# micropilot/myosuite-mjx

Measured on AMD Instinct MI355X. Metric: env-steps/s (whole node) myoHandPoseRandom-v0 batch 4096, higher is better.
Workload: dtype f32

## Files before the change

### myosuite_mjx_amd/csrc/myo_kernel_wave.h

```cpp
#ifndef MYO_KERNEL_WAVE_H
#define MYO_KERNEL_WAVE_H

#define NCONW 32
#define MPRW 14
static_assert(4 * MPRW <= 63, "the scheduler carries the table in a 64-word row (word 63 = entry count)");
struct LayW {
  int qpos, qvel, act, ctrl, lpos, lmat, axis, anchor, xv, qfc, sq, mprw, X;
  int tJ, tlen, tforce;
  int cdof, cinert, crb, cvel, cacc, cfrc;
  int gpos, gax, cand, cdist, cpos, cnrm, cpair, cJ, cdofs;
  int Mp;
  int tJp;
  int total;
};
__host__ __device__ constexpr LayW layout_w(int nq, int nv, int nu, int nl, int ngt, int maxnnz, int ncg, bool has_tl, int nvt, int kc, int nc, int nj) {
  LayW Y{};
  int o = 0;
  Y.qpos = o; o += nq; Y.qvel = o; o += nv; Y.act = o; o += nu; Y.ctrl = o; o += nu;
  Y.lpos = o; o += 3 * nl; Y.lmat = o; o += 9 * nl; Y.axis = o; o += 3 * nv; Y.anchor = o; o += 3 * nv;
  Y.xv = o; o += nvt; Y.qfc = o; o += nvt; Y.sq = o; o += nvt * (nvt + 1); Y.mprw = o; o += 4 * MPRW;
  Y.tJp = 0;
  if (has_tl) { Y.tJp = o; o += ngt * maxnnz + 2 * ngt; }
  Y.X = o;
  Y.tJ = o; o += ngt * maxnnz; Y.tlen = o; o += ngt; Y.tforce = o; o += nu;
  const int endT = o;
  o = Y.X;
  Y.cdof = o; o += 6 * nv; Y.cinert = o; o += 10 * nl; Y.crb = o; o += 10 * nl; Y.cvel = o; o += 6 * nl; Y.cacc = o; o += 6 * nl; Y.cfrc = o; o += 6 * nl;
  const int endD = o;
  o = Y.X;
  Y.Mp = o;
  Y.gpos = o; o += 3 * ncg; Y.gax = o; o += 3 * ncg;
  Y.cand = o; o += NCAND;
  if (o - Y.Mp < (nvt * (nvt + 1)) / 2) o = Y.Mp + (nvt * (nvt + 1)) / 2;
  Y.cdist = o; o += nc; Y.cpos = o; o += 3 * nc; Y.cnrm = o; o += 3 * nc; Y.cpair = o; o += nc;
  Y.cJ = o; o += nc * nj * kc; Y.cdofs = o; o += nc * ((kc + 3) / 4);
  if (o < endT) o = endT;
  if (o < endD) o = endD;
  Y.total = o;
  return Y;
}
struct HfDev { int on, nrow, ncol, cg; float size[4], pos[3]; };
struct DevModelW {
  LayW lay;
  gpi seg_order, seg_tendon, gt_dl;
  gpf link_mat0;
  int nwrapseg, ndl, has_tl;
  gpf tl;
  int nq, has_free, neq;
  int has_j0;
  gpf gt_j0;
  HfDev hf;
  gpi link_free, dof_qposadr, eq_i, link_chain_adr, link_chain;
  int kin_dnmax;
  gpi kin_base, kin_adr, kin_vec;
  gpf eq_f;
  gpf mesh_rec, mesh_startrec, mesh_aabb;
  gpf fl, mesh_vert;
  gpf4 seg_rec;
  gpi dl_pk;
  gpf4 cg_rec;
  gpf4 pair_rec;
  gpi pair_dl_pk;
  gpi kin_pk;
  int kin_nround;
  gpi link_desc;
  gpi link_adof;
  gpi dof_anc;
  unsigned int free_rot[2], free_j3[2];
};
#define SEGR 9
#ifndef MPR_TOL
#define MPR_TOL 1e-8f
#endif

__device__ __forceinline__ float rdlane(float v, int l) { return __int_as_float(__builtin_amdgcn_readlane(__float_as_int(v), l)); }
__device__ __forceinline__ int rdlanei(int v, int l) { return __builtin_amdgcn_readlane(v, l); }
__device__ __forceinline__ float uniformf(float v) { return __int_as_float(__builtin_amdgcn_readfirstlane(__float_as_int(v))); }
template <int CTRL> __device__ __forceinline__ float dpp_add(float v) {
  return v + __int_as_float(__builtin_amdgcn_update_dpp(0, __float_as_int(v), CTRL, 0xf, 0xf, true));
}
__device__ __forceinline__ float wave_sum(float v) {
  v = dpp_add<0xB1>(v);
  v = dpp_add<0x4E>(v);
  v = dpp_add<0x141>(v);
  v = dpp_add<0x140>(v);
  return (rdlane(v, 0) + rdlane(v, 16)) + (rdlane(v, 32) + rdlane(v, 48));
}
#define WFOR(i, n) for (int i = lane; i < (n); i += 64)
__device__ __forceinline__ int wave_lane() {
  int l;
  asm volatile("v_mbcnt_lo_u32_b32 %0, -1, 0\n\tv_mbcnt_hi_u32_b32 %0, -1, %0" : "=v"(l));
  return l;
}
#define CDOF(E_, Y_, c_, k_) ((int)((((const unsigned int*)((E_) + (Y_).cdofs))[CDW * (c_) + ((k_) >> 2)] >> (8 * ((k_) & 3))) & 255u))
#define CDOFP(W_, k_) ((int)(((W_)[(k_) >> 2] >> (8 * ((k_) & 3))) & 255u))

template <int NVT> __device__ __forceinline__ float chol_rows(float (&r)[NVT], int lane) {
  float invd = 1.0f;
#pragma unroll
  for (int j = 0; j < NVT; j++) {
    const float pj = fmaxf(rdlane(r[j], j), MINVALF);
    const float ip = __builtin_amdgcn_rcpf(pj);
    const float col = lane > j ? r[j] : 0.f;
    const float lt = col * ip;
    r[j] = lt;
    if (lane == j) invd = ip;
#pragma unroll
    for (int k = j + 1; k < NVT; k++) r[k] -= lt * rdlane(col, k);
  }
  return invd;
}
template <int SPEC> struct SpecTree { static constexpr int nv = 0; static constexpr int parent[1] = {-1}; };
template <> struct SpecTree<1> { static constexpr int nv = 23;
  static constexpr int parent[23] = {-1, 0, 1, 2, 3, 4, 5, 2, 7, 8, 9, 2, 11, 12, 13, 2, 15, 16, 17, 2, 19, 20, 21}; };
template <> struct SpecTree<2> { static constexpr int nv = 34;
  static constexpr int parent[34] = {-1, 0, 1, 2, 3, 4, 5, 6, 7, 8, 9, 10, 11, 12, 13, 14, 15, 8, 17, 18, 5, 20, 21, 22, 23, 24, 25, 26, 27, 28, 29, 22, 31, 32}; };
template <> struct SpecTree<3> : SpecTree<2> {};
template <int SPEC> __host__ __device__ constexpr bool tree_anc(int a, int d) {
  int p = SpecTree<SPEC>::parent[d];
  while (p >= 0) { if (p == a) return true; p = SpecTree<SPEC>::parent[p]; }
  return false;
}
template <int NVT, int SPEC, int J, int K> __device__ __forceinline__ void tree_update(float (&r)[NVT], float lt, float col) {
  constexpr int nv = SpecTree<SPEC>::nv;
  if constexpr (K > J && J < nv && K < nv) {
    if constexpr (tree_anc<SPEC>(nv - 1 - K, nv - 1 - J)) r[K] -= lt * rdlane(col, K);
  }
}
template <int NVT, int SPEC, int J, int... Ks> __device__ __forceinline__ void tree_col(float (&r)[NVT], float lt, float col, std::integer_sequence<int, Ks...>) {
  (tree_update<NVT, SPEC, J, Ks>(r, lt, col), ...);
}
template <int NVT, int SPEC, int J> __device__ __forceinline__ void tree_step(float (&r)[NVT], float& invd, int lane) {
  const float pj = fmaxf(rdlane(r[J], J), MINVALF);
  const float ip = __builtin_amdgcn_rcpf(pj);
  const float col = lane > J ? r[J] : 0.f;
  const float lt = col * ip;
  r[J] = lt;
  if (lane == J) invd = ip;
  tree_col<NVT, SPEC, J>(r, lt, col, std::make_integer_sequence<int, NVT>{});
}
template <int NVT, int SPEC, int... Js> __device__ __forceinline__ void tree_all(float (&r)[NVT], float& invd, int lane, std::integer_sequence<int, Js...>) {
  (tree_step<NVT, SPEC, Js>(r, invd, lane), ...);
}
template <int NVT, int SPEC> __device__ __forceinline__ float chol_rows_tree(float (&r)[NVT], int lane) {
  float invd = 1.0f;
  tree_all<NVT, SPEC>(r, invd, lane, std::make_integer_sequence<int, NVT>{});
  return invd;
}
template <int NVT> __device__ __forceinline__ float chol_solve_rows(const float (&r)[NVT], float invd, float b, const float* T, int lane) {
  float y = b;
#pragma unroll
  for (int j = 0; j < NVT; j++) y = fmaf(-r[j], rdlane(y, j), y);
  y *= invd;
  const float* Tc = T + (lane < NVT ? lane : 0);
#pragma unroll
  for (int j = NVT - 1; j >= 0; j--) y = fmaf(-Tc[j * (NVT + 1)], rdlane(y, j), y);
  return y;
}
template <int NVT> __device__ __forceinline__ float symv_lds(const float* Mp, float x, int lane, int nv) {
  float s = 0;
  const int d = lane < nv ? lane : 0;
  const int based = (d * (d + 1)) / 2;
#pragma unroll
  for (int k = 0; k < NVT; k++) {
    int kk = k < nv ? k : 0;
    int adr = (kk <= d) ? based + kk : (kk * (kk + 1)) / 2 + d;
    float mv = (k < nv && lane < nv) ? Mp[adr] : 0.f;
    s += mv * rdlane(x, k);
  }
// ... 1179 lines not shown
          lD = __builtin_amdgcn_rcpf(R);
        }
      }
    }
    float caref[NR], cD = 0.f, cmu = 0.f;
#pragma unroll
    for (int k = 0; k < NR; k++) caref[k] = 0.f;
    float cmut = 0.f, cD2 = 0.f;
    int ckc = 0;
    constexpr int ROWS = 8 + NJ * KC + CDW;
    enum { S_AREF = 0, S_D = NR, S_MU = NR + 1, S_MUT = NR + 2, S_D2 = NR + 3, S_KC = NR + 4, S_JAR = NR + 5, S_JV = 2 * NR + 5, S_FC = 3 * NR + 5, S_HC = 3 * NR + 9, S_SIG = 3 * NR + 16 };
    static_assert(!TRK || 3 * NR + 17 <= TRK_STATE, "state block of a second-bank contact");
    const bool bank1 = TRK && ncon > 64;
    auto st1 = [&](int c) -> float* { return ovf_env + (size_t)(c - NC) * ovf_row + ROWS; };
    const bool b1lane = bank1 && lane + 64 < ncon;
    int nefc_b1 = 0;
    auto build_row = [&](const float* pdist, const float* ppos, const float* pnrm, const int* ppair, float* cJ, unsigned int* cdw) {
      const int cw_ = ppair[0], p = cw_ & 2047;
      const float4 pq0_ = W.pair_rec[4 * (size_t)(p)]; const int pw_ = __float_as_int(pq0_.x); const int P[6] = {pw_ & 255, (pw_ >> 8) & 255, (int)((unsigned int)cw_ >> 16), (cw_ >> 11) & 31, (pw_ >> 16) & 15, (pw_ >> 20) & 15};
      const float* F = M.pair_f + 12 * p;
      float n[3] = {pnrm[0], pnrm[1], pnrm[2]}, t1[3], t2[3];
      float cp[3] = {ppos[0], ppos[1], ppos[2]};
      make_frame(n, t1, t2);
      if (FULL && P[4] == 2) {
        const float* ax = E + Y.gax + 3 * P[1];
        float t = dot3(ax, n), y[3] = {ax[0] - t * n[0], ax[1] - t * n[1], ax[2] - t * n[2]};
        float yn = norm3(y);
        if (yn >= 0.5f) {
          float inv = 1.0f / yn;
          t1[0] = y[0] * inv; t1[1] = y[1] * inv; t1[2] = y[2] * inv;
          cross3(t2, n, t1);
        }
      }
      float vn = 0, vt1 = 0, vt2 = 0, vs = 0;
      unsigned int dpk[CDW];
#pragma unroll
      for (int k = 0; k < CDW; k++) dpk[k] = 0;
      ckc = P[3];
#pragma unroll
      for (int k = 0; k < KC; k++) {
        float jn = 0, j1 = 0, j2 = 0, js = 0;
        int d = 0;
        if (k < ckc) {
          const int de_ = W.pair_dl_pk[P[2] + k];
          d = de_ & 127;
          float sg = (float)(de_ >> 8);
          const float* ax = E + Y.axis + 3 * d;
          float col[3];
          if (de_ & 128) {
            float r[3] = {cp[0] - E[Y.anchor + 3 * d], cp[1] - E[Y.anchor + 3 * d + 1], cp[2] - E[Y.anchor + 3 * d + 2]};
            cross3(col, ax, r);
          } else { col[0] = ax[0]; col[1] = ax[1]; col[2] = ax[2]; }
          jn = sg * dot3(n, col); j1 = sg * dot3(t1, col); j2 = sg * dot3(t2, col);
          float qv = E[Y.qvel + d];
          vn += jn * qv; vt1 += j1 * qv; vt2 += j2 * qv;
          if constexpr (TRK) { js = (de_ & 128) ? sg * dot3(n, ax) : 0.f; vs += js * qv; }
        }
        cJ[k] = jn; cJ[KC + k] = j1; cJ[2 * KC + k] = j2;
        if constexpr (TRK) cJ[3 * KC + k] = js;
        dpk[k >> 2] |= (unsigned int)d << (8 * (k & 3));
      }
#pragma unroll
      for (int k = 0; k < CDW; k++) cdw[k] = dpk[k];
      float dist = pdist[0], incl = F[0] - F[1];
      cmu = F[2];
      float imp = impedance(F + 6, dist, incl), K, B;
      kbi(F[4], F[5], F[7], M.timestep, &K, &B);
      if (FULL && P[5] == 1) {
        cmu = 0.f;
        cD = 0.25f / fmaxf(MINVALF, (1 - imp) / imp * F[3]);
      } else {
        float R0 = fmaxf(MINVALF, (1 - imp) / imp * F[3] * (1 + cmu * cmu));
        cD = __builtin_amdgcn_rcpf(fmaxf(MINVALF, 2 * cmu * cmu * R0));
      }
      float pos = -K * imp * (dist - incl);
      caref[0] = -B * (vn + cmu * vt1) + pos; caref[1] = -B * (vn - cmu * vt1) + pos;
      caref[2] = -B * (vn + cmu * vt2) + pos; caref[3] = -B * (vn - cmu * vt2) + pos;
      if constexpr (TRK) {
        if (P[5] == 4) { cmut = F[11]; cD2 = cD; caref[4] = -B * (vn + cmut * vs) + pos; caref[5] = -B * (vn - cmut * vs) + pos; }
      }
    };
    if constexpr (KC == 8 && !FULL && !TRK) {
      float vn_c = 0.f, vt1_c = 0.f, vt2_c = 0.f;
      const int rg = lane >> 3, rk = lane & 7;
      for (int c0 = 0; c0 < ncon; c0 += 8) {
        const int c = c0 + rg;
        float pv0 = 0.f, pv1 = 0.f, pv2 = 0.f;
        auto row_cols = [&](const float* ppos, const float* pnrm, const int* ppair, float* cJ, unsigned int* cdw) {
          const int cw_ = ppair[0];
          const int P[4] = {0, 0, (int)((unsigned int)cw_ >> 16), (cw_ >> 11) & 31};
          const float n[3] = {pnrm[0], pnrm[1], pnrm[2]}, cp[3] = {ppos[0], ppos[1], ppos[2]};
          float t1[3], t2[3];
          make_frame(n, t1, t2);
          float jn = 0.f, j1 = 0.f, j2 = 0.f;
          int d = 0;
          if (rk < P[3]) {
            const int de_ = W.pair_dl_pk[P[2] + rk];
            d = de_ & 127;
            const float sg = (float)(de_ >> 8);
            const float* ax = E + Y.axis + 3 * d;
            float col[3];
            if (de_ & 128) {
              const float r[3] = {cp[0] - E[Y.anchor + 3 * d], cp[1] - E[Y.anchor + 3 * d + 1], cp[2] - E[Y.anchor + 3 * d + 2]};
              cross3(col, ax, r);
            } else { col[0] = ax[0]; col[1] = ax[1]; col[2] = ax[2]; }
            jn = sg * dot3(n, col); j1 = sg * dot3(t1, col); j2 = sg * dot3(t2, col);
            const float qv = E[Y.qvel + d];
            pv0 = jn * qv; pv1 = j1 * qv; pv2 = j2 * qv;
          }
          cJ[rk] = jn; cJ[KC + rk] = j1; cJ[2 * KC + rk] = j2;
          ((unsigned char*)cdw)[rk] = (unsigned char)d;
        };
        if (c < ncon) {
          if (c < NC) row_cols(E + Y.cpos + 3 * c, E + Y.cnrm + 3 * c, (const int*)(E + Y.cpair) + c, E + Y.cJ + c * NJ * KC, (unsigned int*)(E + Y.cdofs) + CDW * c);
          else { float* g = ovf_env + (c - NC) * ovf_row; row_cols(g + 1, g + 4, (const int*)g + 7, g + 8, (unsigned int*)(g + 8 + NJ * KC)); }
        }
#pragma unroll
        for (int m_ = 1; m_ < 8; m_ <<= 1) { pv0 += __shfl_xor(pv0, m_); pv1 += __shfl_xor(pv1, m_); pv2 += __shfl_xor(pv2, m_); }
        const int src = (8 * (lane - c0)) & 63;
        const float a0 = __shfl(pv0, src), a1 = __shfl(pv1, src), a2 = __shfl(pv2, src);
        if (lane >= c0 && lane < c0 + 8) { vn_c = a0; vt1_c = a1; vt2_c = a2; }
      }
      SYNC();
      if (lane < ncon) {
        const float* g = lane < NC ? nullptr : ovf_env + (lane - NC) * ovf_row;
        const int cw_ = lane < NC ? ((const int*)(E + Y.cpair))[lane] : ((const int*)g)[7], p = cw_ & 2047;
        const float dist = lane < NC ? E[Y.cdist + lane] : g[0];
        const float* F = M.pair_f + 12 * p;
        ckc = (cw_ >> 11) & 31;
        const float incl = F[0] - F[1];
        cmu = F[2];
        float imp = impedance(F + 6, dist, incl), K, B;
        kbi(F[4], F[5], F[7], M.timestep, &K, &B);
        const float R0 = fmaxf(MINVALF, (1 - imp) / imp * F[3] * (1 + cmu * cmu));
        cD = __builtin_amdgcn_rcpf(fmaxf(MINVALF, 2 * cmu * cmu * R0));
        const float pos = -K * imp * (dist - incl);
        caref[0] = -B * (vn_c + cmu * vt1_c) + pos; caref[1] = -B * (vn_c - cmu * vt1_c) + pos;
        caref[2] = -B * (vn_c + cmu * vt2_c) + pos; caref[3] = -B * (vn_c - cmu * vt2_c) + pos;
      }
    } else if constexpr (KC == 20) {
      const int rg = lane / KC, rk = lane - rg * KC;
      float vn_c = 0.f, vt1_c = 0.f, vt2_c = 0.f, vs_c = 0.f;
      float vn_1 = 0.f, vt1_1 = 0.f, vt2_1 = 0.f, vs_1 = 0.f;
      for (int c0 = 0; c0 < ncon; c0 += 3) {
        if (lane < 12) E[Y.xv + lane] = 0.f;
        SYNC();
        const int c = c0 + rg;
        auto row_cols = [&](const float* ppos, const float* pnrm, const int* ppair, float* cJ, unsigned int* cdw) {
          const int cw_ = ppair[0];
          const float4 pq0_ = W.pair_rec[4 * (size_t)(cw_ & 2047)]; const int pw_ = __float_as_int(pq0_.x); const int P[6] = {pw_ & 255, (pw_ >> 8) & 255, (int)((unsigned int)cw_ >> 16), (cw_ >> 11) & 31, (pw_ >> 16) & 15, (pw_ >> 20) & 15};
          const float n[3] = {pnrm[0], pnrm[1], pnrm[2]}, cp[3] = {ppos[0], ppos[1], ppos[2]};
          float t1[3], t2[3];
          make_frame(n, t1, t2);
          if (P[4] == 2) {
            const float* ax = E + Y.gax + 3 * P[1];
            float t = dot3(ax, n), y[3] = {ax[0] - t * n[0], ax[1] - t * n[1], ax[2] - t * n[2]};
            float yn = norm3(y);
            if (yn >= 0.5f) {
              float inv = 1.0f / yn;
              t1[0] = y[0] * inv; t1[1] = y[1] * inv; t1[2] = y[2] * inv;
              cross3(t2, n, t1);
            }
          }
          float jn = 0.f, j1 = 0.f, j2 = 0.f, js = 0.f;
          int d = 0;
          if (rk < P[3]) {
            const int de_ = W.pair_dl_pk[P[2] + rk];
            d = de_ & 127;
            const float sg = (float)(de_ >> 8);
            const float* ax = E + Y.axis + 3 * d;
            float col[3];
            const bool hinge = (de_ & 128) != 0;
            if (hinge) {
              const float r[3] = {cp[0] - E[Y.anchor + 3 * d], cp[1] - E[Y.anchor + 3 * d + 1], cp[2] - E[Y.anchor + 3 * d + 2]};
              cross3(col, ax, r);
            } else { col[0] = ax[0]; col[1] = ax[1]; col[2] = ax[2]; }
            jn = sg * dot3(n, col); j1 = sg * dot3(t1, col); j2 = sg * dot3(t2, col);
            const float qv = E[Y.qvel + d];
            atomicAdd(&E[Y.xv + 4 * rg], jn * qv); atomicAdd(&E[Y.xv + 4 * rg + 1], j1 * qv); atomicAdd(&E[Y.xv + 4 * rg + 2], j2 * qv);
            if constexpr (TRK) { js = hinge ? sg * dot3(n, ax) : 0.f; atomicAdd(&E[Y.xv + 4 * rg + 3], js * qv); }
          }
          cJ[rk] = jn; cJ[KC + rk] = j1; cJ[2 * KC + rk] = j2;
          if constexpr (TRK) cJ[3 * KC + rk] = js;
          ((unsigned char*)cdw)[rk] = (unsigned char)d;
        };
        if (rg < 3 && c < ncon) {
          if (c < NC) row_cols(E + Y.cpos + 3 * c, E + Y.cnrm + 3 * c, (const int*)(E + Y.cpair) + c, E + Y.cJ + c * NJ * KC, (unsigned int*)(E + Y.cdofs) + CDW * c);
          else { float* g = ovf_env + (c - NC) * ovf_row; row_cols(g + 1, g + 4, (const int*)g + 7, g + 8, (unsigned int*)(g + 8 + NJ * KC)); }
        }
        SYNC();
        if (lane >= c0 && lane < c0 + 3) { const int g = lane - c0; vn_c = E[Y.xv + 4 * g]; vt1_c = E[Y.xv + 4 * g + 1]; vt2_c = E[Y.xv + 4 * g + 2]; vs_c = E[Y.xv + 4 * g + 3]; }
        if constexpr (TRK) {
          if (b1lane && lane + 64 >= c0 && lane + 64 < c0 + 3) { const int g = lane + 64 - c0; vn_1 = E[Y.xv + 4 * g]; vt1_1 = E[Y.xv + 4 * g + 1]; vt2_1 = E[Y.xv + 4 * g + 2]; vs_1 = E[Y.xv + 4 * g + 3]; }
        }
        SYNC();
      }
      auto row_consts = [&](const int cc, const float vn_c, const float vt1_c, const float vt2_c, const float vs_c, float (&caref)[NR], float& cD, float& cmu, float& cmut,
                            float& cD2, int& ckc) {
        const int lane = cc;
        const float* g = lane < NC ? nullptr : ovf_env + (lane - NC) * ovf_row;
        const int cw_ = lane < NC ? ((const int*)(E + Y.cpair))[lane] : ((const int*)g)[7], p = cw_ & 2047;
        const float dist = lane < NC ? E[Y.cdist + lane] : g[0];
        const float4 pq0_ = W.pair_rec[4 * (size_t)(p)]; const int pw_ = __float_as_int(pq0_.x); const int P[6] = {pw_ & 255, (pw_ >> 8) & 255, __float_as_int(pq0_.w), (pw_ >> 24) & 255, (pw_ >> 16) & 15, (pw_ >> 20) & 15};
// ... 76 lines not shown
        }
      }
      unsigned long long bal = __ballot(tact);
      int slot = nt + __popcll(bal & ((1ull << lane) - 1ull));
      const int ntcap = min(nct, 64);
      if (tact && slot < ntcap) {
        float* const row = slot < NC ? nullptr : ovf_env + (slot - NC) * ovf_row;
        float* cJ = slot < NC ? E + Y.cJ + slot * NJ * KC : row + 8;
        unsigned int dpk[CDW];
#pragma unroll
        for (int k = 0; k < CDW; k++) dpk[k] = 0;
        int kc = 0;
#pragma unroll
        for (int k = 0; k < KC; k++) {
          int d = k < maxnnz_ ? M.gt_dofs[gt * maxnnz_ + k] : -1;
          float jv = d >= 0 ? t_sign * E[Y.tJp + gt * maxnnz_ + k] : 0.f;
          if (d >= 0) kc = k + 1; else d = 0;
          cJ[k] = jv; cJ[KC + k] = 0.f; cJ[2 * KC + k] = 0.f;
          if constexpr (TRK) cJ[3 * KC + k] = 0.f;
          dpk[k >> 2] |= (unsigned int)d << (8 * (k & 3));
        }
        unsigned int* const dw = slot < NC ? (unsigned int*)(E + Y.cdofs) + CDW * slot : (unsigned int*)(row + 8 + NJ * KC);
#pragma unroll
        for (int k = 0; k < CDW; k++) dw[k] = dpk[k];
        if (slot < NC) { E[Y.cdist + slot] = t_aref; E[Y.cpos + 3 * slot] = t_D; E[Y.cpos + 3 * slot + 1] = (float)kc; }
        else { row[0] = t_aref; row[1] = t_D; row[2] = (float)kc; }
      }
      nt += __popcll(bal);
      }
      if (nt > min(nct, 64)) { flags |= MYO_FLAG_CONTACT_OVERFLOW; nt = min(nct, 64); }
      SYNC();
      if (lane >= ncon && lane < nt) {
        const float* const row = lane < NC ? nullptr : ovf_env + (lane - NC) * ovf_row;
        const float a = lane < NC ? E[Y.cdist + lane] : row[0];
        caref[0] = caref[1] = caref[2] = caref[3] = a;
        cD = 0.25f * (lane < NC ? E[Y.cpos + 3 * lane] : row[1]); cmu = 0.f; ckc = (int)(lane < NC ? E[Y.cpos + 3 * lane + 1] : row[2]);
      }
      nefc += nt - ncon;
      ncon = nt;
    }
    float eJ2 = 0.f, eD = 0.f, earef = 0.f, ejar = 0.f, ejv = 0.f;
    int ed1 = 0, ed2 = 0;
    const bool eact = lane < neq;
    if (eact) {
      const int* Q = W.eq_i + 4 * lane;
      const float* F = W.eq_f + 16 * lane;
      ed1 = Q[0]; ed2 = Q[1];
      float x = E[Y.qpos + Q[3]] - F[6];
      float pos = E[Y.qpos + Q[2]] - F[5] - (F[0] + x * (F[1] + x * (F[2] + x * (F[3] + x * F[4]))));
      eJ2 = -(F[1] + x * (2 * F[2] + x * (3 * F[3] + x * 4 * F[4])));
      float vel = E[Y.qvel + ed1] + eJ2 * E[Y.qvel + ed2];
      float imp = impedance(F + 9, pos, 0.f), K, B;
      kbi(F[7], F[8], F[10], M.timestep, &K, &B);
      earef = -B * vel - K * imp * pos;
      eD = __builtin_amdgcn_rcpf(fmaxf(MINVALF, (1 - imp) / imp * F[14]));
    }
    nefc += neq;
    SYNC();
#ifdef MYO_NO_MROW
    constexpr bool MROW = false;
#else
    constexpr bool MROW = NVT > 24 && !RK4;
#endif
    float mrow[MROW ? NVT : 1];
    if constexpr (MROW) {
      const int ml = lane < nv ? lane : 0;
#pragma unroll
      for (int k = 0; k < NVT; k++) mrow[k] = lane < nv ? E[Y.sq + ml * (NVT + 1) + k] : 0.f;
    }
    if (lane < nv) {
      const int based = (lane * (lane + 1)) / 2;
#pragma unroll
      for (int k = 0; k < NVT; k++) if (k <= lane) E[Y.Mp + based + k] = E[Y.sq + lane * (NVT + 1) + k];
    }
    const float* Mp = E + Y.Mp;
    auto symv_reg = [&](float x, int lane) -> float {
      if constexpr (MROW) {
        float s0 = 0.f, s1 = 0.f;
#pragma unroll
        for (int k = 0; k < NVT; k += 2) { s0 = fmaf(mrow[k], rdlane(x, k), s0); if (k + 1 < NVT) s1 = fmaf(mrow[k + 1], rdlane(x, k + 1), s1); }
        return s0 + s1;
      } else return symv_lds<NVT>(Mp, x, lane, nv);
    };
    SYNC();
    STAMP(5);
    SUB0();
    float Ma = 0.f, grad = 0.f, qfc = 0.f, ljar = 0.f, ljv = 0.f, cost = 0.f, qaccE = 0.f, qacc = 0.f;
    float cjar[NR], cjv[NR];
#pragma unroll
    for (int k = 0; k < NR; k++) { cjar[k] = 0.f; cjv[k] = 0.f; }
    int phase = nefc > 0 ? 0 : 1, iters = 0;
    if (phase == 0) {
      qacc = warm_r;
      Ma = symv_reg(qacc, lane);
      ljar = lsign * qacc - laref;
      if constexpr (TRK) fljar = qacc - flaref;
      if (lane < nv) E[Y.xv + lane] = qacc;
      SYNC();
      auto row_jar = [&](const float* cJ, const unsigned int* cdw) {
        float an = 0, a1 = 0, a2 = 0, a3 = 0;
#pragma unroll
        for (int k = 0; k < KC; k++) {
          float xv = E[Y.xv + CDOFP(cdw, k)]; an += cJ[k] * xv; a1 += cJ[KC + k] * xv; a2 += cJ[2 * KC + k] * xv;
          if constexpr (TRK) a3 += cJ[3 * KC + k] * xv;
        }
        cjar[0] = an + cmu * a1 - caref[0]; cjar[1] = an - cmu * a1 - caref[1]; cjar[2] = an + cmu * a2 - caref[2]; cjar[3] = an - cmu * a2 - caref[3];
        if constexpr (TRK) { cjar[4] = an + cmut * a3 - caref[4]; cjar[5] = an - cmut * a3 - caref[5]; }
      };
      if (lane < ncon) {
        if (lane < NC) row_jar(E + Y.cJ + lane * NJ * KC, (const unsigned int*)(E + Y.cdofs) + CDW * lane);
        else { const float* g = ovf_env + (lane - NC) * ovf_row; row_jar(g + 8, (const unsigned int*)(g + 8 + NJ * KC)); }
      }
      if constexpr (TRK) {
        if (b1lane) {
          const float* g = ovf_env + (lane + 64 - NC) * ovf_row;
          const unsigned int* cdw = (const unsigned int*)(g + 8 + NJ * KC);
          float* S = st1(lane + 64);
          float an = 0, a1 = 0, a2 = 0, a3 = 0;
          for (int k = 0; k < KC; k++) { const float xv = E[Y.xv + CDOFP(cdw, k)]; an += g[8 + k] * xv; a1 += g[8 + KC + k] * xv; a2 += g[8 + 2 * KC + k] * xv; a3 += g[8 + 3 * KC + k] * xv; }
          const float mu = S[S_MU], mut = S[S_MUT];
          S[S_JAR] = an + mu * a1 - S[S_AREF]; S[S_JAR + 1] = an - mu * a1 - S[S_AREF + 1]; S[S_JAR + 2] = an + mu * a2 - S[S_AREF + 2]; S[S_JAR + 3] = an - mu * a2 - S[S_AREF + 3];
          S[S_JAR + 4] = an + mut * a3 - S[S_AREF + 4]; S[S_JAR + 5] = an - mut * a3 - S[S_AREF + 5];
        }
      }
      if (eact) ejar = E[Y.xv + ed1] + eJ2 * E[Y.xv + ed2] - earef;
    }
    SUB(6);
    bool first = true;
    int sig_prev = -1;
    while (true) {
      const int lane = wave_lane();
      float r[NVT], rhs, invd;
      bool refactor = true;
      if (phase == 0) {
        bool lact = lsign != 0.f && ljar < 0;
        float w0 = cjar[0] < 0 ? cD : 0.f, w1 = cjar[1] < 0 ? cD : 0.f, w2 = cjar[2] < 0 ? cD : 0.f, w3 = cjar[3] < 0 ? cD : 0.f;
        float f0 = -w0 * cjar[0], f1 = -w1 * cjar[1], f2 = -w2 * cjar[2], f3 = -w3 * cjar[3];
        float w4 = 0.f, w5 = 0.f, f4 = 0.f, f5 = 0.f, flforce = 0.f, flcost = 0.f;
        bool flquad = false;
        if constexpr (TRK) {
          w4 = cjar[4] < 0 ? cD2 : 0.f; w5 = cjar[5] < 0 ? cD2 : 0.f;
          f4 = -w4 * cjar[4]; f5 = -w5 * cjar[5];
          if (flf > 0.f) {
            if (fljar <= -flrf) { flforce = flf; flcost = flf * (-0.5f * flrf - fljar); }
            else if (fljar >= flrf) { flforce = -flf; flcost = flf * (-0.5f * flrf + fljar); }
            else { flforce = -flD * fljar; flcost = 0.5f * flD * fljar * fljar; flquad = true; }
          }
        }
        float cst_b1 = 0.f;
        bool sig_b1_changed = false;
        if constexpr (TRK) {
          if (b1lane) {
            float* S = st1(lane + 64);
            const float D = S[S_D], D2 = S[S_D2], mu = S[S_MU], mut = S[S_MUT];
            float w[NR], f[NR];
            int sg = 0;
#pragma unroll
            for (int k = 0; k < NR; k++) {
              const float jr = S[S_JAR + k];
              w[k] = jr < 0 ? (k < 4 ? D : D2) : 0.f;
              f[k] = -w[k] * jr;
              cst_b1 += 0.5f * w[k] * jr * jr;
              sg |= (w[k] != 0.f ? 2 : 0) << k;
            }
            S[S_FC] = f[0] + f[1] + f[2] + f[3] + f[4] + f[5]; S[S_FC + 1] = mu * (f[0] - f[1]); S[S_FC + 2] = mu * (f[2] - f[3]); S[S_FC + 3] = mut * (f[4] - f[5]);
            S[S_HC] = w[0] + w[1] + w[2] + w[3] + w[4] + w[5]; S[S_HC + 1] = mu * (w[0] - w[1]); S[S_HC + 2] = mu * (w[2] - w[3]);
            S[S_HC + 3] = mu * mu * (w[0] + w[1]); S[S_HC + 4] = mu * mu * (w[2] + w[3]); S[S_HC + 5] = mut * (w[4] - w[5]); S[S_HC + 6] = mut * mut * (w[4] + w[5]);
            sig_b1_changed = ((const int*)S)[S_SIG] != sg;
            ((int*)S)[S_SIG] = sg;
          }
        }
        if (lane < nv) E[Y.qfc + lane] = (lact ? -lsign * lD * ljar : 0.f) + flforce;
        SYNC();
        if constexpr (KC == 8 || TRK) {
          const float Fn = f0 + f1 + f2 + f3 + f4 + f5, Ft1 = cmu * (f0 - f1), Ft2 = cmu * (f2 - f3), Ft3 = cmut * (f4 - f5);
          constexpr int FG = 64 / KC;
          const int fg = lane / KC, fk = lane - fg * KC;
          for (int c0 = 0; c0 < ncon; c0 += FG) {
            const int c = c0 + fg;
            const bool on = fg < FG && c < ncon;
            const int cs = on ? c : 0;
            float sFn = __shfl(Fn, cs & 63), sF1 = __shfl(Ft1, cs & 63), sF2 = __shfl(Ft2, cs & 63), sF3 = TRK ? __shfl(Ft3, cs & 63) : 0.f;
            int kc = __shfl(ckc, cs & 63);
            if constexpr (TRK) {
              if (on && c >= 64) { const float* S = st1(c); sFn = S[S_FC]; sF1 = S[S_FC + 1]; sF2 = S[S_FC + 2]; sF3 = S[S_FC + 3]; kc = ((const int*)S)[S_KC]; }
            }
            if (on && fk < kc) {
              if (c < NC) {
                const float* cJ = E + Y.cJ + c * NJ * KC;
                atomicAdd(&E[Y.qfc + CDOF(E, Y, c, fk)], sFn * cJ[fk] + sF1 * cJ[KC + fk] + sF2 * cJ[2 * KC + fk] + (TRK ? sF3 * cJ[(NJ - 1) * KC + fk] : 0.f));
              } else {
                const float* cJ = ovf_env + (c - NC) * ovf_row + 8;
                const unsigned int* cdw = (const unsigned int*)(cJ + NJ * KC);
                atomicAdd(&E[Y.qfc + CDOFP(cdw, fk)], sFn * cJ[fk] + sF1 * cJ[KC + fk] + sF2 * cJ[2 * KC + fk] + (TRK ? sF3 * cJ[(NJ - 1) * KC + fk] : 0.f));
// ... 100 lines not shown
            if (eact) {
              atomicAdd(&E[Y.sq + ed1 * (NVT + 1) + ed1], eD);
              atomicAdd(&E[Y.sq + ed2 * (NVT + 1) + ed2], eD * eJ2 * eJ2);
              atomicAdd(&E[Y.sq + max(ed1, ed2) * (NVT + 1) + min(ed1, ed2)], eD * eJ2);
            }
            SYNC();
          }
        }
        first = false;
        SUB(1);
      }
      rhs = phase == 0 ? -grad : (phase == 1 ? smooth : smooth + qfc);
      float x;
#ifndef MYO_NO_TREE
#define MYO_NO_TREE 0
#endif
      if (SPEC != 0 && !RK4 && phase != 0 && !MYO_NO_TREE) {
        constexpr int NVS = SpecTree<SPEC>::nv > 0 ? SpecTree<SPEC>::nv : 1;
        const bool act = lane < NVS;
        const int q = act ? NVS - 1 - lane : 0;
        const float dadd = phase == 2 ? h * M.dof_damping[q] : 0.f;
        const float rhs_p = act ? __shfl(rhs, q) : 0.f;
#pragma unroll
        for (int k = 0; k < NVT; k++) {
          const int qk = k < NVS ? NVS - 1 - k : 0;
          const float mv = (act && k <= lane) ? Mp[(qk * (qk + 1)) / 2 + q] : 0.f;
          r[k] = act ? mv + (k == lane ? dadd : 0.f) : (k == lane ? 1.f : 0.f);
        }
        SYNC();
        invd = chol_rows_tree<NVT, SPEC>(r, lane);
        if (lane < NVT) {
#pragma unroll
          for (int k = 0; k < NVT; k++) E[Y.sq + lane * (NVT + 1) + k] = r[k];
          E[Y.sq + lane * (NVT + 1) + NVT] = invd;
        }
        SYNC();
        SUB(2);
        const float xp = chol_solve_rows<NVT>(r, invd, rhs_p, E + Y.sq, lane);
        x = __shfl(xp, act ? NVS - 1 - lane : lane);
      } else {
      if (refactor) {
        if (phase == 0) {
          const int ll_ = lane < NVT ? lane : 0;
#pragma unroll
          for (int k = 0; k < NVT; k++) r[k] = lane < NVT ? E[Y.sq + ll_ * (NVT + 1) + k] : 0.f;
        } else {
          const int dd = lane < nv ? lane : 0;
          const int based = (dd * (dd + 1)) / 2;
          const float diag_add = (phase == 2 && !RK4) ? h * M.dof_damping[dd] : 0.f;
#pragma unroll
          for (int k = 0; k < NVT; k++) {
            float mv;
            if constexpr (MROW) mv = (k <= lane) ? mrow[k] : 0.f;
            else mv = (lane < nv && k <= lane) ? Mp[based + (k <= dd ? k : 0)] : 0.f;
            r[k] = (lane < nv) ? mv + (k == lane ? diag_add : 0.f) : (k == lane ? 1.f : 0.f);
          }
        }
        SYNC();
        invd = chol_rows<NVT>(r, lane);
        if (lane < NVT) {
#pragma unroll
          for (int k = 0; k < NVT; k++) E[Y.sq + lane * (NVT + 1) + k] = r[k];
          E[Y.sq + lane * (NVT + 1) + NVT] = invd;
        }
        SYNC();
      } else {
        const int ll = lane < NVT ? lane : 0;
#pragma unroll
        for (int k = 0; k < NVT; k++) r[k] = E[Y.sq + ll * (NVT + 1) + k];
        invd = E[Y.sq + ll * (NVT + 1) + NVT];
      }
      SUB(2);
      x = chol_solve_rows<NVT>(r, invd, rhs, E + Y.sq, lane);
      }
      SUB(3);
      if (phase == 1) { qacc = x; qfc = 0.f; phase = 2; continue; }
      if (phase == 2) { qaccE = x; break; }
      float search = lane < nv ? x : 0.f;
      float Mv = symv_reg(search, lane);
      ljv = lsign * search;
      if constexpr (TRK) fljv = search;
      if (lane < nv) E[Y.xv + lane] = search;
      SYNC();
      auto row_jv = [&](const float* cJ, const unsigned int* cdw) {
        float an = 0, a1 = 0, a2 = 0, a3 = 0;
#pragma unroll
        for (int k = 0; k < KC; k++) {
          float xv = E[Y.xv + CDOFP(cdw, k)]; an += cJ[k] * xv; a1 += cJ[KC + k] * xv; a2 += cJ[2 * KC + k] * xv;
          if constexpr (TRK) a3 += cJ[3 * KC + k] * xv;
        }
        cjv[0] = an + cmu * a1; cjv[1] = an - cmu * a1; cjv[2] = an + cmu * a2; cjv[3] = an - cmu * a2;
        if constexpr (TRK) { cjv[4] = an + cmut * a3; cjv[5] = an - cmut * a3; }
      };
      if (lane < ncon) {
        if (lane < NC) row_jv(E + Y.cJ + lane * NJ * KC, (const unsigned int*)(E + Y.cdofs) + CDW * lane);
        else { const float* g = ovf_env + (lane - NC) * ovf_row; row_jv(g + 8, (const unsigned int*)(g + 8 + NJ * KC)); }
      }
      if constexpr (TRK) {
        if (b1lane) {
          const float* g = ovf_env + (lane + 64 - NC) * ovf_row;
          const unsigned int* cdw = (const unsigned int*)(g + 8 + NJ * KC);
          float* S = st1(lane + 64);
          float an = 0, a1 = 0, a2 = 0, a3 = 0;
          for (int k = 0; k < KC; k++) { const float xv = E[Y.xv + CDOFP(cdw, k)]; an += g[8 + k] * xv; a1 += g[8 + KC + k] * xv; a2 += g[8 + 2 * KC + k] * xv; a3 += g[8 + 3 * KC + k] * xv; }
          const float mu = S[S_MU], mut = S[S_MUT];
          S[S_JV] = an + mu * a1; S[S_JV + 1] = an - mu * a1; S[S_JV + 2] = an + mu * a2; S[S_JV + 3] = an - mu * a2; S[S_JV + 4] = an + mut * a3; S[S_JV + 5] = an - mut * a3;
        }
      }
      if (eact) ejv = E[Y.xv + ed1] + eJ2 * E[Y.xv + ed2];
      float g1 = wave_sum(search * (Ma - smooth)), g2 = wave_sum(0.5f * search * Mv), sn = sqrtf(wave_sum(search * search));
      SUB(4);
      float alpha = 0, lo = 0, hi = -1, dlo = 0, d2lo = 0, dhi = 0, d2hi = 0, d1init = 0;
      bool ls_on = sn >= MINVALF;
      for (int lsit = -1; lsit < M.ls_iterations && ls_on; lsit++) {
        float a = (lsit < 0) ? 0.f : alpha;
        float p1 = 0, p2 = 0;
        if (lsign != 0.f) { float xx = ljar + a * ljv; if (xx < 0) { p1 += lD * xx * ljv; p2 += lD * ljv * ljv; } }
        p1 += eD * (ejar + a * ejv) * ejv; p2 += eD * ejv * ejv;
#pragma unroll
        for (int k = 0; k < 4; k++) { float xx = cjar[k] + a * cjv[k]; if (xx < 0) { p1 += cD * xx * cjv[k]; p2 += cD * cjv[k] * cjv[k]; } }
        if constexpr (TRK) {
#pragma unroll
          for (int k = 4; k < 6; k++) { float xx = cjar[k] + a * cjv[k]; if (xx < 0) { p1 += cD2 * xx * cjv[k]; p2 += cD2 * cjv[k] * cjv[k]; } }
          if (flf > 0.f) {
            const float xx = fljar + a * fljv;
            if (xx <= -flrf) p1 -= flf * fljv;
            else if (xx >= flrf) p1 += flf * fljv;
            else { p1 += flD * xx * fljv; p2 += flD * fljv * fljv; }
          }
          if (b1lane) {
            const float* S = st1(lane + 64);
            const float D = S[S_D], D2 = S[S_D2];
#pragma unroll
            for (int k = 0; k < NR; k++) { const float jv = S[S_JV + k], xx = S[S_JAR + k] + a * jv, Dk = k < 4 ? D : D2; if (xx < 0) { p1 += Dk * xx * jv; p2 += Dk * jv * jv; } }
          }
        }
        const float sp1 = wave_sum(p1);
        float d1 = sp1 + g1 + 2 * a * g2;
        float d2 = wave_sum(p2) + 2 * g2;
        if (lsit < 0) {
          if (d1 >= 0 || d2 <= 0) { ls_on = false; alpha = 0; break; }
          dlo = d1; d2lo = d2; d1init = fabsf(d1);
          alpha = -d1 / d2;
          continue;
        }
        f_ls++;
        float gtol = fmaxf(fmaxf(M.tolerance * M.ls_tolerance * sn / M.newton_scale, LS_FLOOR * d1init), LS_NOISE * (fabsf(g1) + fabsf(2 * a * g2) + fabsf(sp1)));
        if (fabsf(d1) < gtol) break;
        if (d1 < 0) { lo = alpha; dlo = d1; d2lo = d2; } else { hi = alpha; dhi = d1; d2hi = d2; }
        float cand = alpha - d1 / d2;
        if (hi < 0) {
          if (!(cand > lo)) break;
          alpha = cand;
        } else {
          if (!(cand > lo && cand < hi)) {
            float c2 = d1 < 0 ? hi - dhi / d2hi : lo - dlo / d2lo;
            cand = (c2 > lo && c2 < hi) ? c2 : 0.5f * (lo + hi);
          }
          if (cand == alpha || hi - lo <= 1e-7f * hi) break;
          alpha = cand;
        }
      }
      SUB(5);
      if (!(alpha > 0)) { phase = 2; continue; }
      qacc += alpha * search; Ma += alpha * Mv; ljar += alpha * ljv; ejar += alpha * ejv;
      if constexpr (TRK) fljar += alpha * fljv;
#pragma unroll
      for (int k = 0; k < NR; k++) cjar[k] += alpha * cjv[k];
      if constexpr (TRK) {
        if (b1lane) {
          float* S = st1(lane + 64);
#pragma unroll
          for (int k = 0; k < NR; k++) S[S_JAR + k] += alpha * S[S_JV + k];
        }
      }
    }
    STAMP(7);
    d_nefc = nefc; d_ncon = ncon_real; d_iter = max(d_iter, iters);
    f_ncon += ncon; f_iter += iters;
// ... 170 lines not shown
```

Baseline: 4.278 million.

## Spread contact Jacobian-vector products across 8 lanes per contact with permlane sums

Adds slot_sum8, which reduces across lanes with the same low-3-bit index using a row_shr DPP step plus permlane16/32 swaps. The contact setup loop now maps contacts to lane&7 and the nonzero slot to lane>>3 so it can use this reduction instead of shuffles. The solver's J·x products for jar and jv are computed by the same 8-lanes-per-contact scheme via a new jx8 helper, replacing one serial loop of 8 iterations per lane. A symv_start variant reads Mrow from the square matrix with readlane broadcasts for the initial Ma. The aim is to shorten the serial per-lane work and remove the ds_bpermute shuffles. In exchange, each block of 8 contacts now costs an extra reduction round, and the DPP row_shr 8 control may not reduce the lanes the way intended.

```diff
diff --git a/myosuite_mjx_amd/csrc/myo_kernel_wave.h b/myosuite_mjx_amd/csrc/myo_kernel_wave.h
--- a/myosuite_mjx_amd/csrc/myo_kernel_wave.h
+++ b/myosuite_mjx_amd/csrc/myo_kernel_wave.h
@@ -85,6 +85,13 @@
   v = dpp_add<0x141>(v);
   v = dpp_add<0x140>(v);
   return (rdlane(v, 0) + rdlane(v, 16)) + (rdlane(v, 32) + rdlane(v, 48));
+}
+__device__ __forceinline__ float slot_sum8(float v) {
+  v = dpp_add<0x128>(v);
+  const auto a = __builtin_amdgcn_permlane16_swap(__float_as_int(v), __float_as_int(v), false, false);
+  v = __int_as_float(a[0]) + __int_as_float(a[1]);
+  const auto b = __builtin_amdgcn_permlane32_swap(__float_as_int(v), __float_as_int(v), false, false);
+  return __int_as_float(b[0]) + __int_as_float(b[1]);
 }
 #define WFOR(i, n) for (int i = lane; i < (n); i += 64)
 __device__ __forceinline__ int wave_lane() {
@@ -1430,7 +1437,7 @@
     };
     if constexpr (KC == 8 && !FULL && !TRK) {
       float vn_c = 0.f, vt1_c = 0.f, vt2_c = 0.f;
-      const int rg = lane >> 3, rk = lane & 7;
+      const int rg = lane & 7, rk = lane >> 3;
       for (int c0 = 0; c0 < ncon; c0 += 8) {
         const int c = c0 + rg;
         float pv0 = 0.f, pv1 = 0.f, pv2 = 0.f;
@@ -1463,10 +1470,7 @@
           if (c < NC) row_cols(E + Y.cpos + 3 * c, E + Y.cnrm + 3 * c, (const int*)(E + Y.cpair) + c, E + Y.cJ + c * NJ * KC, (unsigned int*)(E + Y.cdofs) + CDW * c);
           else { float* g = ovf_env + (c - NC) * ovf_row; row_cols(g + 1, g + 4, (const int*)g + 7, g + 8, (unsigned int*)(g + 8 + NJ * KC)); }
         }
-#pragma unroll
-        for (int m_ = 1; m_ < 8; m_ <<= 1) { pv0 += __shfl_xor(pv0, m_); pv1 += __shfl_xor(pv1, m_); pv2 += __shfl_xor(pv2, m_); }
-        const int src = (8 * (lane - c0)) & 63;
-        const float a0 = __shfl(pv0, src), a1 = __shfl(pv1, src), a2 = __shfl(pv2, src);
+        const float a0 = slot_sum8(pv0), a1 = slot_sum8(pv1), a2 = slot_sum8(pv2);
         if (lane >= c0 && lane < c0 + 8) { vn_c = a0; vt1_c = a1; vt2_c = a2; }
       }
       SYNC();
@@ -1709,6 +1713,16 @@
         return s0 + s1;
       } else return symv_lds<NVT>(Mp, x, lane, nv);
     };
+    auto symv_start = [&](float x, int lane) -> float {
+      if constexpr (MROW) return symv_reg(x, lane);
+      else {
+        const float* Mr = E + Y.sq + (lane < nv ? lane : 0) * (NVT + 1);
+        float s = 0.f;
+#pragma unroll
+        for (int k = 0; k < NVT; k++) s += (k < nv ? Mr[k] : 0.f) * rdlane(x, k);
+        return lane < nv ? s : 0.f;
+      }
+    };
     SYNC();
     STAMP(5);
     SUB0();
@@ -1717,13 +1731,35 @@
 #pragma unroll
     for (int k = 0; k < NR; k++) { cjar[k] = 0.f; cjv[k] = 0.f; }
     int phase = nefc > 0 ? 0 : 1, iters = 0;
+    auto jx8 = [&](float& an_, float& a1_, float& a2_, int lane) {
+      const int g = lane & 7, s = lane >> 3;
+      for (int c0 = 0; c0 < ncon; c0 += 8) {
+        const int c = c0 + g;
+        float pn = 0.f, p1 = 0.f, p2 = 0.f;
+        auto jcol = [&](const float* cJ, const unsigned int* cdw) {
+          const float xv = E[Y.xv + CDOFP(cdw, s)];
+          pn = cJ[s] * xv; p1 = cJ[KC + s] * xv; p2 = cJ[2 * KC + s] * xv;
+        };
+        if (c < ncon) {
+          if (c < NC) jcol(E + Y.cJ + c * NJ * KC, (const unsigned int*)(E + Y.cdofs) + CDW * c);
+          else { const float* gr = ovf_env + (c - NC) * ovf_row; jcol(gr + 8, (const unsigned int*)(gr + 8 + NJ * KC)); }
+        }
+        const float sn = slot_sum8(pn), s1 = slot_sum8(p1), s2 = slot_sum8(p2);
+        if (lane >= c0 && lane < c0 + 8) { an_ = sn; a1_ = s1; a2_ = s2; }
+      }
+    };
     if (phase == 0) {
       qacc = warm_r;
-      Ma = symv_reg(qacc, lane);
+      Ma = symv_start(qacc, lane);
       ljar = lsign * qacc - laref;
       if constexpr (TRK) fljar = qacc - flaref;
       if (lane < nv) E[Y.xv + lane] = qacc;
       SYNC();
+      if constexpr (KC == 8 && !TRK) {
+        float an = 0.f, a1 = 0.f, a2 = 0.f;
+        jx8(an, a1, a2, lane);
+        if (lane < ncon) { cjar[0] = an + cmu * a1 - caref[0]; cjar[1] = an - cmu * a1 - caref[1]; cjar[2] = an + cmu * a2 - caref[2]; cjar[3] = an - cmu * a2 - caref[3]; }
+      } else {
       auto row_jar = [&](const float* cJ, const unsigned int* cdw) {
         float an = 0, a1 = 0, a2 = 0, a3 = 0;
 #pragma unroll
@@ -1737,6 +1773,7 @@
       if (lane < ncon) {
         if (lane < NC) row_jar(E + Y.cJ + lane * NJ * KC, (const unsigned int*)(E + Y.cdofs) + CDW * lane);
         else { const float* g = ovf_env + (lane - NC) * ovf_row; row_jar(g + 8, (const unsigned int*)(g + 8 + NJ * KC)); }
+      }
       }
       if constexpr (TRK) {
         if (b1lane) {
@@ -2003,6 +2040,11 @@
       if constexpr (TRK) fljv = search;
       if (lane < nv) E[Y.xv + lane] = search;
       SYNC();
+      if constexpr (KC == 8 && !TRK) {
+        float an = 0.f, a1 = 0.f, a2 = 0.f;
+        jx8(an, a1, a2, lane);
+        if (lane < ncon) { cjv[0] = an + cmu * a1; cjv[1] = an - cmu * a1; cjv[2] = an + cmu * a2; cjv[3] = an - cmu * a2; }
+      } else {
       auto row_jv = [&](const float* cJ, const unsigned int* cdw) {
         float an = 0, a1 = 0, a2 = 0, a3 = 0;
 #pragma unroll
@@ -2016,6 +2058,7 @@
       if (lane < ncon) {
         if (lane < NC) row_jv(E + Y.cJ + lane * NJ * KC, (const unsigned int*)(E + Y.cdofs) + CDW * lane);
         else { const float* g = ovf_env + (lane - NC) * ovf_row; row_jv(g + 8, (const unsigned int*)(g + 8 + NJ * KC)); }
+      }
       }
       if constexpr (TRK) {
         if (b1lane) {
```

Measured after the change: 4.287 million (median of 6 runs). About the same (+0.2%).
